# lukeshope/hipims-ocl

Measured on AMD Instinct MI355X. Metric: Mcell-steps/sec fp64 Godunov+HLLC, 4096^2 grid, 1/2/4/8 MI355X; % HBM roofline, higher is better.
Workload: dtype f64

## Files before the change

hipims-ocl_amd/csrc/hp_engine.hip:

```cpp
#include "hp_domain.hpp"
#include "hp_observers.hpp"
#include "hp_actors.hpp"
#include <hip/hip_ext.h>
#include <dlfcn.h>

#include <algorithm>
#include <cmath>
#include <cstdio>
#include <cstdlib>
#include <cstring>
#include <random>
#include <string>
#include <vector>
#include <unistd.h>

namespace {

constexpr size_t CFL_SLOT_BYTES = 1024;

struct Rccl {
	void* handle = nullptr;
	decltype(&ncclGetUniqueId)   GetUniqueId = nullptr;
	decltype(&ncclCommInitRank)  CommInitRank = nullptr;
	decltype(&ncclCommDestroy)   CommDestroy = nullptr;
// ... 2 lines not shown
	decltype(&ncclSend)          Send = nullptr;
	decltype(&ncclRecv)          Recv = nullptr;
	decltype(&ncclAllReduce)     AllReduce = nullptr;
	decltype(&ncclGetErrorString) GetErrorString = nullptr;
	decltype(&ncclCommCount)     CommCount = nullptr;
	std::string path;
} g_rccl;

void peer_release(hp_domain* d);
PeerBox peer_box(hp_domain* d, bool use, long timeout_ms = 0);
PeerPush make_push(const hp_domain* d);

const PlanKnobs& plan_knobs()
{
	static const PlanKnobs knobs = [] {
		auto num = [](const char* name, int unset) { const char* e = std::getenv(name); return e ? std::atoi(e) : unset; };
		auto off = [&](const char* name) { return num(name, 1) == 0; };
		auto on = [&](const char* name) { return num(name, 0) != 0; };
		auto force = [&](const char* name) { return std::getenv(name) ? (num(name, 0) != 0 ? 1 : 0) : -1; };
		PlanKnobs k;
		k.two_step = num("HP_TWO_STEP", -1);
		k.launch_tail = !off("HP_LAUNCH_TAIL"); k.strip_reduce_always = on("HP_STRIP_REDUCE_ALWAYS");
		k.pair_bdy = !off("HP_PAIR_BDY"); k.pair_strict = !off("HP_PAIR_STRICT"); k.pair_exact = force("HP_PAIR_EXACT");
		k.pair_skip = !off("HP_PAIR_SKIP"); k.fill_after_pairs = !off("HP_FILL_AFTER_PAIRS");
		k.strict_speculate = on("HP_STRICT_SPECULATE"); k.pair_tune = !off("HP_PAIR_TUNE"); k.sweep_alternate = force("HP_SWEEP_ALTERNATE");
		k.tail_max_blocks = (unsigned)num("HP_TAIL_MAX_BLOCKS", (int)TAIL_MAX_BLOCKS);
		k.tail_max_blocks_k2k6 = (unsigned)num("HP_TAIL_MAX_BLOCKS_K2K6", (int)TAIL_MAX_BLOCKS);
		k.march2_rseg_forced = std::getenv("HP_MARCH2_RSEG") != nullptr;
		k.fuse_bdy = !off("HP_FUSE_BDY");
		return k;
	}();
	return knobs;
}
PlanDomain plan_domain(const hp_domain* d)
{
	PlanDomain p;
	p.scheme = d->desc.scheme; p.kernel = d->desc.kernel; p.math_mode = d->desc.math_mode; p.precision = d->desc.precision; p.dynamic_dt = d->desc.dynamic_dt;
	p.quirks = d->desc.quirks; p.rows = d->desc.rows; p.cols = d->desc.cols; p.cells = d->cells;
	p.row_offset = d->desc.row_offset; p.global_rows = d->desc.global_rows; p.ghost_rows = d->ghost_rows;
	p.has_bdy = !d->bdy.empty(); p.fusable = d->fusable; p.bdy_on_ring = d->bdy_on_ring;
	for (const Boundary& b : d->bdy)
		if ((b.kind == BDY_UNIFORM && b.definition == HP_UNIFORM_LOSS_RATE) || (b.kind == BDY_GRIDDED && b.definition == HP_GRIDDED_MASS_FLUX)) p.bdy_removes_water = true;
	p.has_comm = d->comm != nullptr; p.comm_world = d->comm_world; p.peer_direct = d->peer_direct; p.peer_mine = d->peer_mine != nullptr;
	p.has_tail_words = d->tail_words != nullptr; p.tail_allowed = d->tail_allowed; p.halo_overlap = d->halo_overlap; p.split_now = d->split_now;
	p.strip_any_bdy = d->strip_any_bdy; p.strip_first = d->strip_first; p.strip_any_full = d->strip_any_full;
	p.spec_now = d->spec_now; p.has_stamps = d->z_state != nullptr; p.march2_pays = d->tiling.march2_pays;
	p.has_links = d->links.groups != 0; p.soil_on = d->soil.on; p.tracer_on = d->tracer.on;
// ... 510 lines not shown
	if ((rc = pair_stamps_alloc(d)) != HP_OK) return rc;
	bool in_place = false;
	if (bdy && !d->facts->m1_valid) {
		if ((rc = pair_cold_start<T>(d)) != HP_OK) return rc;
		in_place = true;
	} else if (bdy) in_place = d->facts->pair_fused_next;
	tail.pair = bdy ? 2 : 1;
	tail.bdy_flag = bdy && followed ? 1 : 0;
	PairAux<T> aux{};
	const bool exact = pair_exact(pd, knobs) && d->z_state != nullptr;
	if (exact) aux.stamps = StampBufs<T>{(char*)d->z_state, d->haz_words};
	aux.prev_gen = d->facts->other_stale ? d->pair_gen : 0u;
	aux.gen = ++d->pair_gen;
	if (aux.gen == 0) aux.gen = ++d->pair_gen;
	aux.list = (const AreaBdyList<T>*)d->fused_list; aux.fuse_next = bdy && followed ? 1 : 0; aux.in_place = in_place ? 1 : 0;
	aux.truncated = (d->desc.quirks & HP_QUIRK_BDY_TRUNCATED) != 0 ? 1 : 0;
	const bool recs = pair_records(pd, knobs, strip, exact, rseg2);
	if (recs) {
		if ((rc = still_rec_alloc(d, tm.nstrips)) != HP_OK) return rc;
		StillRec* const base = (StillRec*)d->still_rec;
		aux.still_out = base + (size_t)(d->still_rec_half ^ 1) * d->still_rec_slots;
		aux.still_in = d->facts->still_rec_valid ? base + (size_t)d->still_rec_half * d->still_rec_slots : nullptr;
		aux.still_rows = d->desc.rows;
	}
	const void* src = d->state[0];
	void* dst = d->state[1];
	const bool sample = d->timing_stride > 0 && d->timing_used < d->timing_events.size() &&
	                    (d->timing_counter++ % (uint64_t)d->timing_stride) == 0;
	if (sample) HIP_TRY(hipEventRecord(d->timing_events[d->timing_used].first, d->stream));
#define HP_LAUNCH_K1B2(CFL_, BDY_, HZ_, TAIL_)                                                                                            \
	hipLaunchKernelGGL((godunov_march2<false, CFL_, BDY_, HZ_, TAIL_, T>), dim3(blocks), dim3(256), 0, d->stream, p, (const Scalars<T>*)d->scalars, \
	                   (const T*)d->bed, (const State4<T>*)src, (State4<T>*)dst, (const T*)d->manning, (T*)d->cfl_slot,                    \
	                   (const T*)d->cfl_slot + SLOT_EDGE, tm, tail, aux)
#define HP_LAUNCH_K1B(CFL_, BDY_, TAIL_) do { if (exact) HP_LAUNCH_K1B2(CFL_, BDY_, true, TAIL_); else HP_LAUNCH_K1B2(CFL_, BDY_, false, TAIL_); } while (0)
	if (d->desc.math_mode == HP_MATH_STRICT)
		hipLaunchKernelGGL((godunov_march2<true, 1, false, true, 1, T>), dim3(blocks), dim3(256), 0, d->stream, p, (const Scalars<T>*)d->scalars,
		                   (const T*)d->bed, (const State4<T>*)src, (State4<T>*)dst, (const T*)d->manning, (T*)d->cfl_slot,
		                   (const T*)d->cfl_slot + SLOT_EDGE, tm, tail, aux);
	else
	if (strip)    { if (d->desc.dynamic_dt) HP_LAUNCH_K1B2(1, false, false, 2); else HP_LAUNCH_K1B2(0, false, false, 2); }
	else if (bdy) HP_LAUNCH_K1B(1, true, 1);
	else          { if (d->desc.dynamic_dt) HP_LAUNCH_K1B(1, false, 1); else HP_LAUNCH_K1B(0, false, 1); }
#undef HP_LAUNCH_K1B
#undef HP_LAUNCH_K1B2
	d->facts.pair_queued(bdy, followed);
	HIP_TRY(hipGetLastError());
// ... 1337 lines not shown
		HIP_TRY(hipEventElapsedTime(&ms, d->timing_events[i].first, d->timing_events[i].second));
		total += std::max(0.0, (double)ms - d->timing_overhead_ms);
		++n;
	}
	*avg_ms = n ? total / n : 0.0;
	*samples = n;
	return HP_OK;
}

int hp_pair_stats(hp_domain_t* d, uint64_t out[12])
{
	int rc = check_domain(d);
	if (rc != HP_OK) return rc;
	if (!out) return fail(HP_ERR_INVALID, "out == NULL");
	out[0] = d->pairs; out[1] = d->pair_cold_starts; out[2] = out[3] = 0;
	HIP_TRY(hipStreamSynchronize(d->stream));
	if (tuner_on(plan_domain(d), plan_knobs()) && (rc = tuner_poll(d)) != HP_OK) return rc;
	out[4] = d->tune_samples; out[5] = d->tune_switches; out[6] = d->tune_prefer_pairs ? 1 : 0;
	out[7] = d->tune_single_ms > 0.f ? (uint64_t)(1000.0 * d->tune_pair_ms / d->tune_single_ms) : 0;
	out[8] = out[9] = out[10] = out[11] = 0;
	if (d->still_rec && d->still_rec_last) {
		const StillRec* half = (const StillRec*)d->still_rec + (size_t)d->still_rec_half * d->still_rec_slots;
		unsigned long long* counts = (unsigned long long*)((StillRec*)d->still_rec + 2 * d->still_rec_slots);
		HIP_TRY(hipMemsetAsync(counts, 0, 16, d->stream));
		hipLaunchKernelGGL(still_rec_count, dim3(256), dim3(256), 0, d->stream, half, d->still_rec_slots, counts);
		HIP_TRY(hipGetLastError());
		unsigned long long host_counts[2] = {0, 0};
		HIP_TRY(hipMemcpyAsync(host_counts, counts, sizeof host_counts, hipMemcpyDeviceToHost, d->stream));
		HIP_TRY(hipStreamSynchronize(d->stream));
		out[9] = host_counts[0]; out[10] = host_counts[1];
	}
	if (d->haz_words) {
		unsigned long long used = 0;
		HIP_TRY(hipMemcpy(&used, d->haz_words + 2, sizeof used, hipMemcpyDeviceToHost));
		out[8] = used;
	}
	if (!d->z_state) return HP_OK;
	unsigned long long* counts = d->haz_words + 4;
	HIP_TRY(hipMemsetAsync(counts, 0, 16, d->stream));
	if (d->desc.precision == 8)
		hipLaunchKernelGGL((stamps_count<double>), dim3(1024), dim3(256), 0, d->stream, StampBufs<double>{(char*)d->z_state, d->haz_words}, d->pair_gen, d->cells, counts);
	else
		hipLaunchKernelGGL((stamps_count<float>), dim3(1024), dim3(256), 0, d->stream, StampBufs<float>{(char*)d->z_state, d->haz_words}, d->pair_gen, d->cells, counts);
	HIP_TRY(hipGetLastError());
	unsigned long long host_counts[2] = {0, 0};
	HIP_TRY(hipMemcpyAsync(host_counts, counts, sizeof host_counts, hipMemcpyDeviceToHost, d->stream));
	HIP_TRY(hipStreamSynchronize(d->stream));
	out[2] = host_counts[0]; out[3] = host_counts[1];
	return HP_OK;
}

int hp_launch_counts(hp_domain_t* d, uint64_t* flux_launches, uint64_t* with_tail)
{
// ... 19 lines not shown
```

hipims-ocl_amd/csrc/hp_kernels.hpp:

```cpp
#pragma once

#include "hp_math.hpp"
#include "hp_tiling.hpp"

namespace hp {

template <bool STRICT, typename T>
__global__ __launch_bounds__(256) void godunov_basic(const Params<T> p, const Scalars<T>* __restrict__ sc,
                                                     const T* __restrict__ bed, const State4<T>* __restrict__ src,
                                                     State4<T>* __restrict__ dst, const T* __restrict__ manning,
                                                     const long y_lo, const long y_hi)
{
	const long x = (long)blockIdx.x * blockDim.x + threadIdx.x;
	const long y = (long)blockIdx.y * blockDim.y + threadIdx.y + y_lo;
	if (x >= p.cols - 1 || y >= y_hi || x <= 0) return;
	const size_t id = (size_t)y * p.cols + x;
	const T dt = sc->dt;

	if (dt <= T(0)) { dst[id] = src[id]; return; }

	const State4<T> c = src[id];
	const T zb = bed[id], n = manning[id];
	if (c.zmax <= T(-9999.0) || c.z == T(-9999.0)) { dst[id] = c; return; }

	const size_t iW = id - 1, iE = id + 1, iS = id - p.cols, iN = id + p.cols;
	const State4<T> cW = src[iW], cE = src[iE], cS = src[iS], cN = src[iN];
// ... 410 lines not shown
}
__device__ __forceinline__ float first_lane(const float v) { return __int_as_float(__builtin_amdgcn_readfirstlane(__float_as_int(v))); }
__device__ __forceinline__ double first_lane(const double v)
{
	return __hiloint2double(__builtin_amdgcn_readfirstlane(__double2hiint(v)), __builtin_amdgcn_readfirstlane(__double2loint(v)));
}
__device__ __forceinline__ unsigned long long value_bits(const double v) { return (unsigned long long)__double_as_longlong(v); }
template <typename V> __device__ __forceinline__ V from_east(const V v) { return lane_move<DPP_WAVE_ROL1>(v); }
template <typename V> __device__ __forceinline__ V from_west(const V v) { return lane_move<DPP_WAVE_ROR1>(v); }

template <typename T> struct RowRegs { State4<T> c; T zb, n; };

template <typename T>
__device__ __forceinline__ Side<T> side_from_east(const Side<T>& s)
{
	Side<T> r;
	r.eta = from_east(s.eta); r.zb = from_east(s.zb);
	r.qx = from_east(s.qx);   r.qy = from_east(s.qy);
	r.u0 = from_east(s.u0);   r.v0 = from_east(s.v0);
	return r;
}


__device__ __forceinline__ bool tile_rows(const TileMap& tm, const int wave, long& strip, long& y0, long& y1)
{
	const unsigned band = blockIdx.x % (unsigned)tm.nbands, i = blockIdx.x / (unsigned)tm.nbands;
	const unsigned nbig_tiles = (unsigned)(tm.groups * tm.nbig);
	const long band_y0 = tm.y_begin + (long)band * tm.band_stride;
	const long band_y1 = (band_y0 + tm.band_rows < tm.y_end) ? (band_y0 + tm.band_rows) : tm.y_end;
	unsigned g;
	long h;
	if (i < nbig_tiles) {
		g = i % (unsigned)tm.groups;
		h = tm.rseg;
		y0 = band_y0 + (long)(i / (unsigned)tm.groups) * tm.rseg;
	} else {
		const unsigned j = i - nbig_tiles;
		g = j % (unsigned)tm.groups;
		h = tm.rseg_tail;
		y0 = band_y0 + (long)tm.nbig * tm.rseg + (long)(j / (unsigned)tm.groups) * tm.rseg_tail;
	}
	y1 = (y0 + h < band_y1) ? (y0 + h) : band_y1;
	strip = (long)g * 4 + wave;
	const bool any = y0 < band_y1 && strip < tm.nstrips;
	if (tm.flip) {
		const long top = band_y0 + (band_y1 - y1);
		y1 = band_y0 + (band_y1 - y0);
		y0 = top;
	}
	return any;
}

template <typename T> struct UniformBdy { const T* series; uint32_t entries; int definition; T interval, length; };
template <typename T> struct GriddedBdy {
	const T* grids; uint64_t entries, grows, gcols; int definition; T resolution, off_x, off_y, interval;
};

template <typename T>
__device__ __forceinline__ bool bdy_in_range(const Params<T>& p, const long x, const long gy, const bool truncated)
{
	if (x >= p.cols - 1 || gy >= p.global_rows - 1 || x <= 0 || gy <= 0) return false;
	if (truncated && (x >= (p.cols / 8) * 8 || gy >= (p.global_rows / 8) * 8)) return false;
	return true;
}

constexpr int AREA_BDY_MAX = 8;
// ... 4 lines not shown
};
template <typename T> struct AreaBdyList { int count; AreaBdy<T> b[AREA_BDY_MAX]; };


constexpr int FUSED_BDY_MAX = 3;
template <typename T> struct FusedBdy {
	T    inc_lo, inc_hi;
	int  y_switch;
	int  mode;
};

template <typename T> constexpr unsigned stamp_rec() { return (unsigned)sizeof(State4<T>) + 16u; }
template <typename T> struct StampBufs { char* rec; unsigned long long* haz; };
template <typename T> __device__ __forceinline__ unsigned stamp_gen(const StampBufs<T>& b, const size_t id)
{
	return *reinterpret_cast<const unsigned*>(b.rec + id * stamp_rec<T>() + sizeof(State4<T>));
}
template <typename T> __device__ __forceinline__ State4<T> stamp_state(const StampBufs<T>& b, const size_t id)
{
	const T* v = reinterpret_cast<const T*>(b.rec + id * stamp_rec<T>());
	State4<T> c; c.z = v[0]; c.zmax = v[1]; c.qx = v[2]; c.qy = v[3];
	return c;
}
struct StillRec { unsigned long long z, b; unsigned tag, pad[3]; };
constexpr unsigned STILL_TAG_RUN = 1, STILL_TAG_SKIP = 2;
template <typename T> struct PairAux {
	StampBufs<T>          stamps;
	unsigned              gen, prev_gen;
	const AreaBdyList<T>* list;
	int                   fuse_next;
	int                   in_place;
	int                   truncated;
	StillRec*             still_out;
	const StillRec*       still_in;
	long                  still_rows;
};

#ifndef HP_K1_STRICT_WAVES
#define HP_K1_STRICT_WAVES 3
#endif
#ifndef HP_K1_FAST_WAVES
#define HP_K1_FAST_WAVES 3
#endif
#ifndef HP_K1_F32_WAVES
#define HP_K1_F32_WAVES 5
#endif
template <bool STRICT, typename T> constexpr int march_waves() { return sizeof(T) == 4 ? HP_K1_F32_WAVES : (STRICT ? HP_K1_STRICT_WAVES : HP_K1_FAST_WAVES); }
// ... 330 lines not shown
template <bool STRICT, int CFL_MODE, bool BDY, bool HZ, int TAIL, typename T>
#ifndef HP_K1B_WAVES_MIN
#define HP_K1B_WAVES_MIN 3
#endif
#ifndef HP_K1B_F32_WAVES_MIN
#define HP_K1B_F32_WAVES_MIN 5
#endif
#ifndef HP_K1B_F32_WAVES_MAX
#define HP_K1B_F32_WAVES_MAX 5
#endif
__global__ __launch_bounds__(256) __attribute__((amdgpu_waves_per_eu(sizeof(T) == 4 ? (STRICT ? 3 : (HZ ? 4 : HP_K1B_F32_WAVES_MIN)) : (STRICT ? HP_K1B_STRICT_WAVES : HP_K1B_WAVES_MIN), sizeof(T) == 4 ? (STRICT ? 3 : HP_K1B_F32_WAVES_MAX) : (STRICT ? HP_K1B_STRICT_WAVES : 3)))) void godunov_march2(
	const Params<T> p, const Scalars<T>* sc, const T* __restrict__ bed, const State4<T>* __restrict__ src,
	State4<T>* __restrict__ dst, const T* __restrict__ manning, T* cfl_slot, const T* __restrict__ edge_max,
	const TileMap tm, const LaunchTail<T> tail, const PairAux<T> aux)
{
	if (TAIL != 0 && blockIdx.x >= tail.flux_blocks) {
		launch_tail(p, tail);
		return;
	}
	__shared__ T inc_tab[BDY ? 4 * 3 * FUSED_BDY_MAX * 2 * 64 : 1];
	const int lane = threadIdx.x & 63, wave = __builtin_amdgcn_readfirstlane((int)(threadIdx.x >> 6));
	long strip, y0, y1;
	T wave_vmax = T(0), wave_vmax1 = T(0);
	if (tile_rows(tm, wave, strip, y0, y1)) {

	const long x = strip * MARCH2_COLS - 1 + lane;
	const long xc = x < 0 ? 0 : (x < p.cols ? x : (p.cols - 1));
	const bool out_x = lane >= 2 && lane <= MARCH2_COLS + 1 && x <= p.cols - 2;
	const bool ring_x = x <= 0 || x >= p.cols - 1;
	const T vs = p.vs;
	const bool with_friction = p.friction != 0;
	const T inv_dx = STRICT ? p.inv_dx_pow2 : p.inv_dx;

	Scalars<T> s1 = *sc;
	const Scalars<T> s0 = s1;
	const T dt_a = s1.dt;
	advance_scalars(p, s1, p.dynamic_dt ? cfl_slot[BDY ? SLOT_M1 : SLOT_SAVED] : T(0));
	const T dt_b = s1.dt;
	const bool skip_a = dt_a <= T(0), skip_b = dt_b <= T(0);
	constexpr bool SCALAR_CONSTS = !STRICT && sizeof(T) == 8;
	constexpr bool HIDE = BDY || HZ;
	const StepConsts<T> ka{uniform_value<HIDE>(-(dt_a * p.inv_dx)), uniform_value<HIDE>(dt_a * gravity<T>()), SCALAR_CONSTS};
	const StepConsts<T> kb{uniform_value<HIDE>(-(dt_b * p.inv_dx)), uniform_value<HIDE>(dt_b * gravity<T>()), SCALAR_CONSTS};

	const long row_base = y0 - 2 < 0 ? 0 : y0 - 2, col_base = strip * MARCH2_COLS - 1 < 0 ? 0 : strip * MARCH2_COLS - 1;
	const size_t cell0 = (size_t)row_base * p.cols + (size_t)col_base;
	const size_t cells_left = (size_t)p.cols * p.rows - cell0;
	const __amdgpu_buffer_rsrc_t srd_src = make_srd(src + cell0, cells_left * sizeof(State4<T>));
	const __amdgpu_buffer_rsrc_t srd_dst = make_srd(dst + cell0, cells_left * sizeof(State4<T>));
	const __amdgpu_buffer_rsrc_t srd_bed = make_srd(bed + cell0, cells_left * sizeof(T));
	const __amdgpu_buffer_rsrc_t srd_man = make_srd(manning + cell0, cells_left * sizeof(T));
	const unsigned lane_col = (unsigned)(xc - col_base);
	const unsigned voff_state = lane_col * (unsigned)sizeof(State4<T>), voff_scalar = lane_col * (unsigned)sizeof(T);
	const unsigned row_state = (unsigned)p.cols * (unsigned)sizeof(State4<T>), row_scalar = (unsigned)p.cols * (unsigned)sizeof(T);
	const long last_row = p.rows - 1;
	const __amdgpu_buffer_rsrc_t srd_peer0 = make_srd((TAIL == 2 && tail.peer_rows[0] ? tail.peer_rows[0] : dst) + cell0, cells_left * sizeof(State4<T>));
	const __amdgpu_buffer_rsrc_t srd_peer1 = make_srd((TAIL == 2 && tail.peer_rows[1] ? tail.peer_rows[1] : dst) + cell0, cells_left * sizeof(State4<T>));
	auto store_peer = [&](const State4<T>& v, const long y, const bool write_lane) {
		const bool e0 = (int)y >= tail.edge_rows[0] && (int)y < tail.edge_rows[1];
		const bool e1 = (int)y >= tail.edge_rows[2] && (int)y < tail.edge_rows[3];
		buf_store_state<HP_AUX_THROUGH>(v, e1 ? srd_peer1 : srd_peer0, (write_lane && (e0 || e1)) ? voff_state : HP_OOB, (unsigned)(y - row_base) * row_state);
	};
	auto load_row = [&](long y, const bool live = true) {
		y = y < 0 ? 0 : (y > last_row ? last_row : y);
		RowRegs<T> r;
		const unsigned k = (unsigned)(y - row_base);
		unsigned vs_ = live ? voff_state : HP_OOB, vc_ = live ? voff_scalar : HP_OOB;
		asm volatile("" : "+v"(vs_), "+v"(vc_));
		r.c = buf_load_state(srd_src, vs_, k * row_state, T());
		r.zb = buf_load_scalar(srd_bed, vc_, k * row_scalar, T());
		r.n = p.manning_uniform ? p.manning_value : buf_load_scalar(srd_man, vc_, k * row_scalar, T());
		return r;
	};
	constexpr bool LAZY_DRY = !STRICT && sizeof(T) == 8;
	auto flux_from_west = [&](const FaceFlux<T>& forW, const bool dryC, bool& dryW) {
		FaceFlux<T> fW;
// ... 68 lines not shown
					if (b.g.definition == 0) {
						inc_lo = rate_lo / T(3600000.0) * thj[j];
						inc_hi = rate_hi / T(3600000.0) * thj[j];
					} else {
						inc_lo = rate_lo / (p.dx * p.dx) * thj[j];
						inc_hi = rate_hi / (p.dx * p.dx) * thj[j];
					}
					ysw[k] = (int)(row_base + n_lo);
					mode = 2u;
				}
				if (mode == 3u) continue;
				tab[((j * FUSED_BDY_MAX + k) * 2 + 0) * 64 + lane] = inc_lo;
				tab[((j * FUSED_BDY_MAX + k) * 2 + 1) * 64 + lane] = inc_hi;
				modes = (modes & ~(3u << (2 * (j * FUSED_BDY_MAX + k)))) | (mode << (2 * (j * FUSED_BDY_MAX + k)));
				act |= 1u << j;
			}
		}
	}
	const bool fuse = BDY && aux.fuse_next != 0;

	T vmax = T(0), vmax1 = T(0);
	unsigned stale_rows = 0;

	constexpr bool RECS = !STRICT && !BDY && !HZ && TAIL == 1 && sizeof(T) == 8;
	unsigned long long still_kz = 0, still_kb = 0;
	unsigned still_marks = 0;
	auto write_recs = [&](const unsigned tag) {
		if (!RECS || aux.still_out == nullptr) return;
		const __amdgpu_buffer_rsrc_t srd = make_srd(aux.still_out + (size_t)strip * aux.still_rows, (size_t)aux.still_rows * sizeof(StillRec));
		const bool m = lane < 32 && ((still_marks >> (unsigned)lane) & 1u) != 0;
		hp_u32x4 a;
		a.x = m ? (unsigned)still_kz : ~0u; a.y = m ? (unsigned)(still_kz >> 32) : ~0u;
		a.z = m ? (unsigned)still_kb : ~0u; a.w = m ? (unsigned)(still_kb >> 32) : ~0u;
		unsigned voff = lane < y1 - y0 ? (unsigned)((y0 + lane) * (long)sizeof(StillRec)) : HP_OOB;
		asm volatile("" : "+v"(voff));
		store_operands_own(a);
		__builtin_amdgcn_raw_buffer_store_b128(a, srd, (int)voff, 0, 0);
		__builtin_amdgcn_raw_buffer_store_b32(m ? tag : 0u, srd, (int)voff + 16, 0, 0);
		store_fence(a, voff, 0u);
	};
	auto tile_known = [&]() -> bool {
		const long xw = strip * MARCH2_COLS - 1;
		if (xw < 1 || xw + 63 > p.cols - 2 || y0 - 2 < 1 || y1 + 1 > last_row - 1 || y1 - y0 > 32) return false;
		const int nr = (int)(y1 - y0) + 4, n = 3 * nr;
		const __amdgpu_buffer_rsrc_t srd = make_srd(aux.still_in + (size_t)(strip - 1) * aux.still_rows, (size_t)3 * aux.still_rows * sizeof(StillRec));
		auto voff = [&](const int i) {
			const int w = i < nr ? 0 : (i < 2 * nr ? 1 : 2);
			return i < n ? (unsigned)(((long)w * aux.still_rows + y0 - 2 + (i - w * nr)) * (long)sizeof(StillRec)) : HP_OOB;
		};
		const hp_u32x4 e0 = __builtin_amdgcn_raw_buffer_load_b128(srd, (int)voff(lane), 0, 0);
		const hp_u32x4 e1 = __builtin_amdgcn_raw_buffer_load_b128(srd, (int)voff(lane + 64), 0, 0);
		const unsigned k0 = __builtin_amdgcn_readfirstlane(e0.x), k1 = __builtin_amdgcn_readfirstlane(e0.y);
		const unsigned k2 = __builtin_amdgcn_readfirstlane(e0.z), k3 = __builtin_amdgcn_readfirstlane(e0.w);
		if (k0 == ~0u && k1 == ~0u) return false;
		auto same = [&](const hp_u32x4& e) { return e.x == k0 && e.y == k1 && e.z == k2 && e.w == k3; };
		if (!wave_all((lane >= n || same(e0)) && (lane + 64 >= n || same(e1)))) return false;
		still_kz = ((unsigned long long)k1 << 32) | k0;
		still_kb = ((unsigned long long)k3 << 32) | k2;
		return true;
	};

// ... 275 lines not shown
			buf_store_state(c, srd_dst, out_x ? voff_state : HP_OOB, row_k * row_state);
			if (TAIL == 2) store_peer(c, yy, out_x);
			if (CFL_MODE == 1 && out_x && (int)yy >= tm.price_lo && (int)yy < tm.price_hi && spd > vmax) vmax = spd;
		};
		State4<T> a = q[2].c, b = q[3].c;
		for (;;) {
			if (y >= y1) return y;
			#pragma unroll
			for (int j = 0; j < 4; ++j) q[j] = load_rz(y + 2 + j);
			if (!in_run(q[0])) return y;
			put(a, y);
			if (y + 1 >= y1 || !in_run(q[1])) return y + 1;
			put(b, y + 1);
			if (y + 2 >= y1 || !in_run(q[2])) return y + 2;
			put(q[0].c, y + 2);
			if (y + 3 >= y1 || !in_run(q[3])) return y + 3;
			put(q[1].c, y + 3);
			a = q[2].c; b = q[3].c;
			y += 4;
		}
	};

	const long yb = (RUNS && !skip_a && !skip_b) ? still_run() : y0;
	write_recs(STILL_TAG_RUN);
	if (!RUNS || yb < y1) {
		prime(yb);
		long r = yb + 1;
		for (; r + 1 <= y1; r += 2) {
			{ const T nn = rc.n; const RowU1<T> u = stage_a(r, rP, rQ); stage_b(r - 1, u, nn, true); }
			{ const T nn = rc.n; const RowU1<T> u = stage_a(r + 1, rQ, rP); stage_b(r, u, nn, true); }
		}
		if (r <= y1) { const T nn = rc.n; const RowU1<T> u = stage_a(r, rP, rQ); stage_b(r - 1, u, nn, true); }
	}

	if (wave_any(stale_rows != 0)) {
		for (long y = y0; y < y1; ++y) {
			if ((stale_rows >> (unsigned)(y - y0)) & 1u) {
				const size_t id = (size_t)y * p.cols + xc;
				const T zb = bed[id];
				State4<T> c = src[id];
				if (live0) c = apply(J0(), c, zb, y);
				State4<T> next = c;
				if (live2) next = apply(J2(), c, zb, y);
				dst[id] = fuse ? next : c;
				if (TAIL == 2) store_peer(fuse ? next : c, y, true);
				if (CFL_MODE == 1 && (int)y >= tm.price_lo && (int)y < tm.price_hi) {
					const T s = cfl_speed<STRICT>(c.z, c.zmax, c.qx, c.qy, zb, p.qs);
					if (s > vmax) vmax = s;
					if (live2) {
						const T s2 = cfl_speed<STRICT>(next.z, next.zmax, next.qx, next.qy, zb, p.qs);
						if (s2 > vmax1) vmax1 = s2;
					}
				}
			}
		}
	}
	if (!live2) vmax1 = vmax;
	};

	auto raise_word = [&]() { if (hz_on && wave_any(stamped) && lane == 0) aux.stamps.haz[aux.gen & 1u] = (unsigned long long)aux.gen; };
	if (RECS && aux.still_in != nullptr && !skip_a && !skip_b && tile_known()) {
		still_marks = ~0u;
		write_recs(STILL_TAG_SKIP);
		if (CFL_MODE == 1 && out_x && (int)y1 > tm.price_lo && (int)y0 < tm.price_hi)
			vmax = cfl_speed<STRICT>(T(__longlong_as_double((long long)still_kz)), T(0), T(0), T(0), T(__longlong_as_double((long long)still_kb)), p.qs);
		vmax1 = vmax;
	} else {
	if (BDY && act != 0) { if (hz_any) march(std::true_type(), std::true_type()); else march(std::true_type(), std::false_type()); }
	else                 { if (hz_any) march(std::false_type(), std::true_type()); else march(std::false_type(), std::false_type()); }
	raise_word();
	}

	if (CFL_MODE != 0) {
		if (blockIdx.x == 0 && wave == 0) { const T e = *edge_max; if (e > vmax) vmax = e; if (e > vmax1) vmax1 = e; }
		vmax = wave_max(vmax);
		if (BDY) vmax1 = wave_max(vmax1);
		if (TAIL != 0) { wave_vmax = vmax; wave_vmax1 = vmax1; }
		else if (lane == 0 && vmax > T(0)) atomic_max_nonneg(cfl_slot, vmax);
	}
	}
	if (TAIL != 0) tail_block_done<BDY>(tail, wave_vmax, wave, lane, y0, y1, wave_vmax1);
}

template <typename T>
__global__ __launch_bounds__(256) void stamps_to_buffer(State4<T>* __restrict__ other, const StampBufs<T> b, const unsigned gen, const size_t cells)
{
	if (b.haz[gen & 1u] != (unsigned long long)gen) return;
	for (size_t id = (size_t)blockIdx.x * blockDim.x + threadIdx.x; id < cells; id += (size_t)gridDim.x * blockDim.x)
		if (stamp_gen(b, id) == gen) other[id] = stamp_state(b, id);
}

template <typename T>
__global__ __launch_bounds__(256) void stamps_count(const StampBufs<T> b, const unsigned gen, const size_t cells, unsigned long long* counts)
{
	unsigned long long last = 0, any = 0;
	for (size_t id = (size_t)blockIdx.x * blockDim.x + threadIdx.x; id < cells; id += (size_t)gridDim.x * blockDim.x) {
		const unsigned g = stamp_gen(b, id);
		last += (g != 0 && g == gen); any += (g != 0);
	}
	for (int off = 32; off > 0; off >>= 1) { last += __shfl_down(last, off); any += __shfl_down(any, off); }
	if ((threadIdx.x & 63) == 0 && (last | any)) { atomicAdd(counts, last); atomicAdd(counts + 1, any); }
}
__global__ __launch_bounds__(256) void still_rec_count(const StillRec* __restrict__ rec, const size_t n, unsigned long long* counts)
{
	unsigned long long skipped = 0, still = 0;
	for (size_t i = (size_t)blockIdx.x * blockDim.x + threadIdx.x; i < n; i += (size_t)gridDim.x * blockDim.x) {
		const unsigned tag = rec[i].tag;
		skipped += (tag == STILL_TAG_SKIP); still += (tag == STILL_TAG_SKIP || tag == STILL_TAG_RUN);
	}
	for (int off = 32; off > 0; off >>= 1) { skipped += __shfl_down(skipped, off); still += __shfl_down(still, off); }
	if ((threadIdx.x & 63) == 0 && (skipped | still)) { atomicAdd(counts, skipped); atomicAdd(counts + 1, still); }
}

template <typename T>
__global__ void pair_cold_start_words(T* slot)
{
	slot[SLOT_M1] = atomic_exchange_zero(slot);
	slot[SLOT_BDY] = T(1);
}

template <typename T>
__global__ __launch_bounds__(256) void rings_compare(const State4<T>* __restrict__ a, const State4<T>* __restrict__ b, const long cols, const long rows,
                                                     unsigned long long* differ)
{
	const long n = 2 * cols + 2 * (rows - 2);
	bool bad = false;
	for (long i = (long)blockIdx.x * blockDim.x + threadIdx.x; i < n; i += (long)gridDim.x * blockDim.x) {
		long x, y;
		if (i < cols) { x = i; y = 0; }
		else if (i < 2 * cols) { x = i - cols; y = rows - 1; }
		else { const long j = i - 2 * cols; x = (j & 1) ? cols - 1 : 0; y = 1 + (j >> 1); }
		const size_t id = (size_t)y * cols + x;
		const unsigned* wa = reinterpret_cast<const unsigned*>(a + id);
		const unsigned* wb = reinterpret_cast<const unsigned*>(b + id);
// ... 606 lines not shown
```

hipims-ocl_amd/csrc/hp_plan.hpp:

```cpp
#pragma once
#include "../../include/hipims_mi.h"
#include "hp_facts.hpp"

#include <algorithm>
#include <cstddef>
#include <cstdint>

namespace hp {
namespace {

constexpr unsigned TAIL_MAX_BLOCKS = 65536;
constexpr uint32_t SPEC_MIN = 8;

struct PlanKnobs {
	int      two_step = -1;
	bool     launch_tail = true;
	bool     strip_reduce_always = false;
	bool     pair_bdy = true;
	bool     pair_strict = true;
	int      pair_exact = -1;
	bool     pair_skip = true;
	bool     fill_after_pairs = true;
	bool     strict_speculate = false;
	bool     pair_tune = true;
	int      sweep_alternate = -1;
	unsigned tail_max_blocks = TAIL_MAX_BLOCKS;
	unsigned tail_max_blocks_k2k6 = TAIL_MAX_BLOCKS;
	bool     march2_rseg_forced = false;
	bool     fuse_bdy = true;
};

struct PlanDomain {
	int      scheme = HP_SCHEME_GODUNOV, kernel = HP_KERNEL_AUTO, math_mode = HP_MATH_FAST, precision = 8, dynamic_dt = 1;
	unsigned quirks = HP_QUIRKS_REFERENCE;
	long     rows = 0, cols = 0;
	size_t   cells = 0;
	long     row_offset = 0, global_rows = 0, ghost_rows = 1;
	bool     has_bdy = false;
	bool     fusable = false, bdy_on_ring = false;
	bool     bdy_removes_water = false;
	bool     has_comm = false;
	int      comm_world = 1;
	bool     peer_direct = false, peer_mine = false;
	bool     has_tail_words = true, tail_allowed = false, halo_overlap = false, split_now = true;
// ... 42 lines not shown
}
inline bool pair_eligible(const PlanDomain& d, const BufferFacts& facts, const PlanKnobs& k)
{
	return pairs_possible(d, k) && facts.pair_ready(d.dynamic_dt != 0);
}
inline bool strip_pairs_possible_here(const PlanDomain& d, const BufferFacts& facts, const PlanKnobs& k)
{
	return pairs_possible_common(d, k) && d.has_comm && d.comm_world > 1 && d.peer_direct && d.ghost_rows == 2 && !facts->rings_differ;
}
inline bool pair_exact(const PlanDomain& d, const PlanKnobs& k)
{
	if (d.math_mode == HP_MATH_STRICT) return true;
	if (k.pair_exact >= 0) return k.pair_exact != 0;
	return d.bdy_removes_water;
}
inline int pair_tile_rows(const PlanDomain& d, const PlanKnobs& k, const int march2_rseg)
{
	return (d.math_mode == HP_MATH_STRICT && !k.march2_rseg_forced) ? std::min(march2_rseg, 12) : march2_rseg;
}
inline bool pair_records(const PlanDomain& d, const PlanKnobs& k, const bool strip, const bool exact, const int tile_rows)
{
	return d.precision == 8 && k.pair_skip && !strip && !d.has_bdy && !exact && d.math_mode != HP_MATH_STRICT && tile_rows <= 32;
}

inline bool fill_wanted(const PlanDomain& d, const BufferFacts& facts, const PlanKnobs& k)
{
	return k.fill_after_pairs && facts->other_stale && d.scheme == HP_SCHEME_GODUNOV && d.kernel != HP_KERNEL_BASIC && !(pair_exact(d, k) && d.has_stamps);
}

inline bool spec_wanted(const PlanDomain& d, const PlanKnobs& k, const uint32_t n)
{
	const bool fusable_ok = d.spec_fused_kept || !d.fusable;
	return k.strict_speculate && n >= SPEC_MIN && d.math_mode == HP_MATH_STRICT && d.precision == 8 && !d.has_comm && fusable_ok && !d.has_links && !d.soil_on && !d.tracer_on &&
	       d.kernel != HP_KERNEL_BASIC && (d.scheme == HP_SCHEME_GODUNOV || d.scheme == HP_SCHEME_MUSCL_HANCOCK);
}
inline bool tuner_on(const PlanDomain& d, const PlanKnobs& k)
{
	return k.pair_tune && d.math_mode == HP_MATH_STRICT && k.two_step != 1;
}

inline bool strips_reduce_everyone(const PlanDomain& d, const BufferFacts& facts, const bool first_of_batch)
{
	const bool dst_is_primary = facts->use_alt == 1;
	return d.dynamic_dt && (d.scheme == HP_SCHEME_MUSCL_HANCOCK || !reads_primary(d) || dst_is_primary || basic_godunov(d) || d.strip_any_bdy ||
	                        (first_of_batch && d.strip_any_full));
}
// ... 44 lines not shown
```

hipims-ocl_amd/csrc/hp_tiling.hpp:

```cpp
#pragma once
#include <algorithm>
#include <cstdlib>
#include <initializer_list>
#include <vector>

namespace hp {

constexpr int MARCH_COLS = 62;
constexpr int MARCH2_COLS = 60;
constexpr int MUSCL_COLS = 60;

struct TileMap {
	int  nstrips, groups;
	long y_begin, y_end;
	int  nbands;
	long band_stride;
	int  band_rows;
	int  rseg, nbig;
	int  rseg_tail, ntail;
	int  price_lo, price_hi;
	int  flip;
};

struct TilingKnobs {
	bool   rseg_refine = true;
	bool   search = true, search_pair = true;
	bool   search_f32 = false;
	double tiling_fill = 3.5, march2_fill = 4.0;
	int    march_rseg = 0, muscl_rseg = 0, inertial_rseg = 0, march2_rseg = 0;
	int    tail_rseg = 0, tail_pct = -1;
	bool   print_tiling = false;
};
struct LaunchKnobs {
	long   halo_rows = 0;
	int    nbands = 0;
};

struct Tiling {
// ... 127 lines not shown
{
	Tiling t = pick_tiling(cols, rows, precision, cus, knobs);
	force_heights(t, knobs);
	return t;
}

inline bool tiles_addressable(const Tiling& t, const long cols, const int precision)
{
	const int rseg_max = std::max(std::max(t.march_rseg, t.march2_rseg), std::max(t.muscl_rseg, t.inertial_rseg));
	return (double)(rseg_max + 4) * (double)cols * 4.0 * (double)precision < 2147483647.0;
}

enum { PART_ALL = 0, PART_HALO = 1, PART_INTERIOR = 2 };

struct RowRange { long lo, hi; };

inline bool make_tile_map(const LaunchKnobs& knobs, long lo, long hi, int g, int part, int nstrips, int rseg, int rseg_tail, int tail_pct,
                          TileMap& tm, unsigned& blocks, int rseg_tall = 16, long need = 0, long price_lo = 0, long price_hi = 0x7fffffffL,
                          int nbands = 8)
{
	if (need < g) need = g;
	const long halo = knobs.halo_rows >= need ? knobs.halo_rows : (rseg > need ? rseg : need);
	tm.price_lo = (int)price_lo; tm.price_hi = (int)(price_hi < 0x7fffffffL ? price_hi : 0x7fffffffL);
	tm.flip = 0;
	const bool can_split = hi - lo > 2 * halo;
	tm.nstrips = nstrips;
	tm.groups = (nstrips + 3) / 4;
	if (part == PART_HALO && can_split) {
		tm.y_begin = lo; tm.y_end = hi;
		tm.nbands = 2; tm.band_stride = (hi - halo) - lo; tm.band_rows = (int)halo;
		tm.rseg = rseg < tm.band_rows ? rseg : tm.band_rows;
		tm.nbig = (tm.band_rows + tm.rseg - 1) / tm.rseg;
		tm.rseg_tail = rseg_tail; tm.ntail = 0;
		blocks = 2u * (unsigned)(tm.groups * tm.nbig);
		return true;
	}
	if (part == PART_INTERIOR) {
		if (!can_split) return false;
		lo += halo; hi -= halo;
	}
	tm.y_begin = lo; tm.y_end = hi;
	const long rows = hi - lo;
	tm.nbands = part != PART_ALL ? 8 : (knobs.nbands >= 1 && knobs.nbands <= 64 ? knobs.nbands : (nbands >= 1 && nbands <= 64 ? nbands : 8));
	tm.band_rows = (int)((rows + tm.nbands - 1) / tm.nbands);
	tm.band_stride = tm.band_rows;
	if (rseg == 16 && g == 1 && tm.band_rows >= 256) rseg = rseg_tall;
	tm.rseg = rseg < tm.band_rows ? rseg : tm.band_rows;
// ... 16 lines not shown
```

hipims-ocl_amd/hipims_mi/__init__.py:

```python
from __future__ import annotations

import ctypes as C
import os
import weakref

import numpy as np

HERE = os.path.dirname(os.path.abspath(__file__))
PKG_ROOT = os.path.dirname(HERE)
LIB_PATH = os.path.join(PKG_ROOT, "lib", "libhipims_mi.so")

SCHEME_GODUNOV, SCHEME_MUSCL_HANCOCK, SCHEME_INERTIAL = 0, 1, 2
ARRAY_STATE, ARRAY_BED, ARRAY_MANNING = 0, 1, 2
QUIRK_CFL_READS_PRIMARY, QUIRK_BDY_TRUNCATED, QUIRK_MUSCL_NEIGHBOUR_Y_IS_BED, QUIRKS_REFERENCE = 1, 2, 4, 7
MATH_FAST, MATH_STRICT = 0, 1
KERNEL_AUTO, KERNEL_BASIC = 0, 1
UNIFORM_RAIN_INTENSITY, UNIFORM_LOSS_RATE = 0, 1
GRIDDED_RAIN_INTENSITY, GRIDDED_RAIN_ACCUMUL, GRIDDED_MASS_FLUX = 0, 1, 2
DEPTH_IGNORE, DEPTH_IS_FSL, DEPTH_IS_DEPTH, DEPTH_IS_CRITICAL = 0, 1, 2, 3
DISCHARGE_IGNORE, DISCHARGE_IS_DISCHARGE, DISCHARGE_IS_VELOCITY, DISCHARGE_IS_VOLUME = 0, 1, 2, 3
PTR_STATE_NEXT_SRC, PTR_STATE_OTHER, PTR_BED, PTR_MANNING, PTR_CFL_MAX, PTR_SCALARS = range(6)
(OUT_DEPTH, OUT_MAXDEPTH, OUT_FSL, OUT_MAXFSL, OUT_DISCHARGE_X, OUT_DISCHARGE_Y, OUT_VELOCITY_X, OUT_VELOCITY_Y, OUT_FROUDE,
 OUT_COUNT) = range(10)
OUT_CODES = {"depth": OUT_DEPTH, "maxdepth": OUT_MAXDEPTH, "fsl": OUT_FSL, "maxfsl": OUT_MAXFSL, "dischargex": OUT_DISCHARGE_X,
# ... 1067 lines not shown
    def kernel_timing(self, stride):
        _check(self.lib, self.lib.hp_kernel_timing(self.h, stride), "hp_kernel_timing")

    def kernel_timing_read(self):
        avg, n = C.c_double(0), C.c_uint32(0)
        _check(self.lib, self.lib.hp_kernel_timing_read(self.h, C.byref(avg), C.byref(n)), "hp_kernel_timing_read")
        return avg.value, n.value

    def launch_counts(self):
        if not hasattr(self.lib, "hp_launch_counts"):
            return None
        a, b = C.c_uint64(0), C.c_uint64(0)
        _check(self.lib, self.lib.hp_launch_counts(self.h, C.byref(a), C.byref(b)), "hp_launch_counts")
        return a.value, b.value

    def pair_stats(self):
        if not hasattr(self.lib, "hp_pair_stats"):
            return None
        out = (C.c_uint64 * 12)()
        self.lib.hp_pair_stats.argtypes = [C.c_void_p, C.POINTER(C.c_uint64)]
        _check(self.lib, self.lib.hp_pair_stats(self.h, out), "hp_pair_stats")
        return dict(pairs=out[0], cold_starts=out[1], stamped_last=out[2], stamped_ever=out[3], tune_samples=out[4],
                    tune_switches=out[5], prefers_pairs=bool(out[6]), pair_over_single=out[7] / 1000.0, stale_used=out[8],
                    skipped_rows=out[9], still_rows=out[10])

    def kernel_timing_overhead(self):
        if not hasattr(self.lib, "hp_kernel_timing_overhead"):
            return 0.0
        ms = C.c_double(0)
        _check(self.lib, self.lib.hp_kernel_timing_overhead(self.h, C.byref(ms)), "hp_kernel_timing_overhead")
        return ms.value

    def depth_velocity(self, state=None, bed=None):
        state = self.download() if state is None else state
        bed = self._bed_host if bed is None else bed
        depth = np.maximum(0.0, state[..., 0].astype(np.float64) - bed.astype(np.float64))
        with np.errstate(divide="ignore", invalid="ignore"):
            u = np.where(depth > 1e-8, state[..., 2] / depth, 0.0)
            v = np.where(depth > 1e-8, state[..., 3] / depth, 0.0)
        return depth, u, v
```

Measured before the change: 122,100.

## Redeal idle waves onto still-marching tiles within a block for skip pairs

When still-water skip records are active, strips are assigned to a block's four waves with a stride instead of contiguously. Waves whose tile was skipped take a share of the rows of the one or two waves that still have to march, splitting those rows into parts of at least three rows. The aim is to cut the load imbalance where a block waits on a single wave marching a full tile. It adds shared-memory flags, extra __syncthreads, recomputed buffer descriptors and a dealt counter in the still records, and it disables still-run marks for split parts, which may cost some skipping.

New measurement: 118,700. 0.972x the previous value.

```diff
diff --git a/hipims-ocl_amd/csrc/hp_engine.hip b/hipims-ocl_amd/csrc/hp_engine.hip
--- a/hipims-ocl_amd/csrc/hp_engine.hip
+++ b/hipims-ocl_amd/csrc/hp_engine.hip
@@ -48,7 +48,7 @@
 		k.two_step = num("HP_TWO_STEP", -1);
 		k.launch_tail = !off("HP_LAUNCH_TAIL"); k.strip_reduce_always = on("HP_STRIP_REDUCE_ALWAYS");
 		k.pair_bdy = !off("HP_PAIR_BDY"); k.pair_strict = !off("HP_PAIR_STRICT"); k.pair_exact = force("HP_PAIR_EXACT");
-		k.pair_skip = !off("HP_PAIR_SKIP"); k.fill_after_pairs = !off("HP_FILL_AFTER_PAIRS");
+		k.pair_skip = !off("HP_PAIR_SKIP"); k.pair_redeal = !off("HP_PAIR_REDEAL"); k.fill_after_pairs = !off("HP_FILL_AFTER_PAIRS");
 		k.strict_speculate = on("HP_STRICT_SPECULATE"); k.pair_tune = !off("HP_PAIR_TUNE"); k.sweep_alternate = force("HP_SWEEP_ALTERNATE");
 		k.tail_max_blocks = (unsigned)num("HP_TAIL_MAX_BLOCKS", (int)TAIL_MAX_BLOCKS);
 		k.tail_max_blocks_k2k6 = (unsigned)num("HP_TAIL_MAX_BLOCKS_K2K6", (int)TAIL_MAX_BLOCKS);
@@ -605,6 +605,7 @@
 		aux.still_out = base + (size_t)(d->still_rec_half ^ 1) * d->still_rec_slots;
 		aux.still_in = d->facts->still_rec_valid ? base + (size_t)d->still_rec_half * d->still_rec_slots : nullptr;
 		aux.still_rows = d->desc.rows;
+		if (pair_redeal(knobs, recs)) tm.stride = tm.groups;
 	}
 	const void* src = d->state[0];
 	void* dst = d->state[1];
@@ -1988,13 +1989,13 @@
 	if (d->still_rec && d->still_rec_last) {
 		const StillRec* half = (const StillRec*)d->still_rec + (size_t)d->still_rec_half * d->still_rec_slots;
 		unsigned long long* counts = (unsigned long long*)((StillRec*)d->still_rec + 2 * d->still_rec_slots);
-		HIP_TRY(hipMemsetAsync(counts, 0, 16, d->stream));
+		HIP_TRY(hipMemsetAsync(counts, 0, 24, d->stream));
 		hipLaunchKernelGGL(still_rec_count, dim3(256), dim3(256), 0, d->stream, half, d->still_rec_slots, counts);
 		HIP_TRY(hipGetLastError());
-		unsigned long long host_counts[2] = {0, 0};
+		unsigned long long host_counts[3] = {0, 0, 0};
 		HIP_TRY(hipMemcpyAsync(host_counts, counts, sizeof host_counts, hipMemcpyDeviceToHost, d->stream));
 		HIP_TRY(hipStreamSynchronize(d->stream));
-		out[9] = host_counts[0]; out[10] = host_counts[1];
+		out[9] = host_counts[0]; out[10] = host_counts[1]; out[11] = host_counts[2];
 	}
 	if (d->haz_words) {
 		unsigned long long used = 0;
diff --git a/hipims-ocl_amd/csrc/hp_kernels.hpp b/hipims-ocl_amd/csrc/hp_kernels.hpp
--- a/hipims-ocl_amd/csrc/hp_kernels.hpp
+++ b/hipims-ocl_amd/csrc/hp_kernels.hpp
@@ -2,6 +2,7 @@
 
 #include "hp_math.hpp"
 #include "hp_tiling.hpp"
+#include "hp_redeal.hpp"
 
 namespace hp {
 
@@ -458,6 +459,7 @@
 }
 
 
+template <bool STRIDED = false>
 __device__ __forceinline__ bool tile_rows(const TileMap& tm, const int wave, long& strip, long& y0, long& y1)
 {
 	const unsigned band = blockIdx.x % (unsigned)tm.nbands, i = blockIdx.x / (unsigned)tm.nbands;
@@ -477,7 +479,7 @@
 		y0 = band_y0 + (long)tm.nbig * tm.rseg + (long)(j / (unsigned)tm.groups) * tm.rseg_tail;
 	}
 	y1 = (y0 + h < band_y1) ? (y0 + h) : band_y1;
-	strip = (long)g * 4 + wave;
+	strip = (STRIDED && tm.stride != 0) ? (long)g + (long)wave * tm.stride : (long)g * 4 + wave;
 	const bool any = y0 < band_y1 && strip < tm.nstrips;
 	if (tm.flip) {
 		const long top = band_y0 + (band_y1 - y1);
@@ -528,7 +530,7 @@
 	State4<T> c; c.z = v[0]; c.zmax = v[1]; c.qx = v[2]; c.qy = v[3];
 	return c;
 }
-struct StillRec { unsigned long long z, b; unsigned tag, pad[3]; };
+struct StillRec { unsigned long long z, b; unsigned tag, dealt, pad[2]; };
 constexpr unsigned STILL_TAG_RUN = 1, STILL_TAG_SKIP = 2;
 template <typename T> struct PairAux {
 	StampBufs<T>          stamps;
@@ -905,12 +907,21 @@
 	const int lane = threadIdx.x & 63, wave = __builtin_amdgcn_readfirstlane((int)(threadIdx.x >> 6));
 	long strip, y0, y1;
 	T wave_vmax = T(0), wave_vmax1 = T(0);
-	if (tile_rows(tm, wave, strip, y0, y1)) {
-
-	const long x = strip * MARCH2_COLS - 1 + lane;
-	const long xc = x < 0 ? 0 : (x < p.cols ? x : (p.cols - 1));
-	const bool out_x = lane >= 2 && lane <= MARCH2_COLS + 1 && x <= p.cols - 2;
-	const bool ring_x = x <= 0 || x >= p.cols - 1;
+	constexpr bool RECS = !STRICT && !BDY && !HZ && TAIL == 1 && sizeof(T) == 8;
+	__shared__ unsigned redeal_words[RECS ? 4 + 16 : 1];
+	const bool have_tile = tile_rows<RECS>(tm, wave, strip, y0, y1);
+	const bool redeal_on = RECS && tm.stride != 0;
+	if (have_tile || redeal_on) {
+
+	long x, xc;
+	bool out_x, ring_x;
+	auto place_columns = [&]() {
+		x = strip * MARCH2_COLS - 1 + lane;
+		xc = x < 0 ? 0 : (x < p.cols ? x : (p.cols - 1));
+		out_x = lane >= 2 && lane <= MARCH2_COLS + 1 && x <= p.cols - 2;
+		ring_x = x <= 0 || x >= p.cols - 1;
+	};
+	place_columns();
 	const T vs = p.vs;
 	const bool with_friction = p.friction != 0;
 	const T inv_dx = STRICT ? p.inv_dx_pow2 : p.inv_dx;
@@ -926,15 +937,22 @@
 	const StepConsts<T> ka{uniform_value<HIDE>(-(dt_a * p.inv_dx)), uniform_value<HIDE>(dt_a * gravity<T>()), SCALAR_CONSTS};
 	const StepConsts<T> kb{uniform_value<HIDE>(-(dt_b * p.inv_dx)), uniform_value<HIDE>(dt_b * gravity<T>()), SCALAR_CONSTS};
 
-	const long row_base = y0 - 2 < 0 ? 0 : y0 - 2, col_base = strip * MARCH2_COLS - 1 < 0 ? 0 : strip * MARCH2_COLS - 1;
-	const size_t cell0 = (size_t)row_base * p.cols + (size_t)col_base;
-	const size_t cells_left = (size_t)p.cols * p.rows - cell0;
-	const __amdgpu_buffer_rsrc_t srd_src = make_srd(src + cell0, cells_left * sizeof(State4<T>));
-	const __amdgpu_buffer_rsrc_t srd_dst = make_srd(dst + cell0, cells_left * sizeof(State4<T>));
-	const __amdgpu_buffer_rsrc_t srd_bed = make_srd(bed + cell0, cells_left * sizeof(T));
-	const __amdgpu_buffer_rsrc_t srd_man = make_srd(manning + cell0, cells_left * sizeof(T));
-	const unsigned lane_col = (unsigned)(xc - col_base);
-	const unsigned voff_state = lane_col * (unsigned)sizeof(State4<T>), voff_scalar = lane_col * (unsigned)sizeof(T);
+	long row_base, col_base;
+	size_t cell0, cells_left;
+	__amdgpu_buffer_rsrc_t srd_src, srd_dst, srd_bed, srd_man;
+	unsigned lane_col, voff_state, voff_scalar;
+	auto place_window = [&]() {
+		row_base = y0 - 2 < 0 ? 0 : y0 - 2; col_base = strip * MARCH2_COLS - 1 < 0 ? 0 : strip * MARCH2_COLS - 1;
+		cell0 = (size_t)row_base * p.cols + (size_t)col_base;
+		cells_left = (size_t)p.cols * p.rows - cell0;
+		srd_src = make_srd(src + cell0, cells_left * sizeof(State4<T>));
+		srd_dst = make_srd(dst + cell0, cells_left * sizeof(State4<T>));
+		srd_bed = make_srd(bed + cell0, cells_left * sizeof(T));
+		srd_man = make_srd(manning + cell0, cells_left * sizeof(T));
+		lane_col = (unsigned)(xc - col_base);
+		voff_state = lane_col * (unsigned)sizeof(State4<T>); voff_scalar = lane_col * (unsigned)sizeof(T);
+	};
+	place_window();
 	const unsigned row_state = (unsigned)p.cols * (unsigned)sizeof(State4<T>), row_scalar = (unsigned)p.cols * (unsigned)sizeof(T);
 	const long last_row = p.rows - 1;
 	const __amdgpu_buffer_rsrc_t srd_peer0 = make_srd((TAIL == 2 && tail.peer_rows[0] ? tail.peer_rows[0] : dst) + cell0, cells_left * sizeof(State4<T>));
@@ -1049,9 +1067,10 @@
 	T vmax = T(0), vmax1 = T(0);
 	unsigned stale_rows = 0;
 
-	constexpr bool RECS = !STRICT && !BDY && !HZ && TAIL == 1 && sizeof(T) == 8;
 	unsigned long long still_kz = 0, still_kb = 0;
 	unsigned still_marks = 0;
+	unsigned redealt = 0;
+	int part_slot = 0, part_index = 0;
 	auto write_recs = [&](const unsigned tag) {
 		if (!RECS || aux.still_out == nullptr) return;
 		const __amdgpu_buffer_rsrc_t srd = make_srd(aux.still_out + (size_t)strip * aux.still_rows, (size_t)aux.still_rows * sizeof(StillRec));
@@ -1064,6 +1083,7 @@
 		store_operands_own(a);
 		__builtin_amdgcn_raw_buffer_store_b128(a, srd, (int)voff, 0, 0);
 		__builtin_amdgcn_raw_buffer_store_b32(m ? tag : 0u, srd, (int)voff + 16, 0, 0);
+		__builtin_amdgcn_raw_buffer_store_b32(redealt, srd, (int)voff + 20, 0, 0);
 		store_fence(a, voff, 0u);
 	};
 	auto tile_known = [&]() -> bool {
@@ -1385,6 +1405,11 @@
 	};
 
 	const long yb = (RUNS && !skip_a && !skip_b) ? still_run() : y0;
+	if (redeal_on) {
+		if (lane == 0) redeal_words[4 + 4 * part_slot + part_index] = yb >= y1 ? 1u : 0u;
+		__syncthreads();
+		for (int j = 0; j < part_index; ++j) if (redeal_words[4 + 4 * part_slot + j] == 0u) still_marks = 0;
+	}
 	write_recs(STILL_TAG_RUN);
 	if (!RUNS || yb < y1) {
 		prime(yb);
@@ -1422,17 +1447,42 @@
 	};
 
 	auto raise_word = [&]() { if (hz_on && wave_any(stamped) && lane == 0) aux.stamps.haz[aux.gen & 1u] = (unsigned long long)aux.gen; };
-	if (RECS && aux.still_in != nullptr && !skip_a && !skip_b && tile_known()) {
+	bool marches = have_tile;
+	if (RECS && have_tile && aux.still_in != nullptr && !skip_a && !skip_b && tile_known()) {
 		still_marks = ~0u;
 		write_recs(STILL_TAG_SKIP);
 		if (CFL_MODE == 1 && out_x && (int)y1 > tm.price_lo && (int)y0 < tm.price_hi)
 			vmax = cfl_speed<STRICT>(T(__longlong_as_double((long long)still_kz)), T(0), T(0), T(0), T(__longlong_as_double((long long)still_kb)), p.qs);
 		vmax1 = vmax;
-	} else {
+		marches = false;
+	}
+	if (redeal_on) {
+		part_slot = wave;
+		if (lane == 0) redeal_words[wave] = (marches ? 1u : 0u) | (have_tile ? 2u : 0u);
+		__syncthreads();
+		if (aux.still_in != nullptr && !skip_a && !skip_b) {
+			unsigned needy = 0, present = 0;
+			for (int w = 0; w < 4; ++w) {
+				const unsigned f = (unsigned)__builtin_amdgcn_readfirstlane((int)redeal_words[w]);
+				needy |= (f & 1u) << (unsigned)w; present |= ((f >> 1) & 1u) << (unsigned)w;
+			}
+			const RedealPart part = redeal_part(needy, present, wave, y0, y1);
+			marches = part.slot >= 0;
+			if (marches && part.parts > 1) {
+				strip += (long)(part.slot - wave) * tm.stride;
+				y0 = part.y0; y1 = part.y1;
+				part_slot = part.slot; part_index = part.part;
+				redealt = 1u; still_marks = 0;
+				place_columns();
+				place_window();
+			}
+		}
+	}
+	if (marches) {
 	if (BDY && act != 0) { if (hz_any) march(std::true_type(), std::true_type()); else march(std::true_type(), std::false_type()); }
 	else                 { if (hz_any) march(std::false_type(), std::true_type()); else march(std::false_type(), std::false_type()); }
 	raise_word();
-	}
+	} else if (redeal_on) __syncthreads();
 
 	if (CFL_MODE != 0) {
 		if (blockIdx.x == 0 && wave == 0) { const T e = *edge_max; if (e > vmax) vmax = e; if (e > vmax1) vmax1 = e; }
@@ -1466,13 +1516,14 @@
 }
 __global__ __launch_bounds__(256) void still_rec_count(const StillRec* __restrict__ rec, const size_t n, unsigned long long* counts)
 {
-	unsigned long long skipped = 0, still = 0;
+	unsigned long long skipped = 0, still = 0, dealt = 0;
 	for (size_t i = (size_t)blockIdx.x * blockDim.x + threadIdx.x; i < n; i += (size_t)gridDim.x * blockDim.x) {
 		const unsigned tag = rec[i].tag;
 		skipped += (tag == STILL_TAG_SKIP); still += (tag == STILL_TAG_SKIP || tag == STILL_TAG_RUN);
-	}
-	for (int off = 32; off > 0; off >>= 1) { skipped += __shfl_down(skipped, off); still += __shfl_down(still, off); }
-	if ((threadIdx.x & 63) == 0 && (skipped | still)) { atomicAdd(counts, skipped); atomicAdd(counts + 1, still); }
+		dealt += (rec[i].dealt == 1u);
+	}
+	for (int off = 32; off > 0; off >>= 1) { skipped += __shfl_down(skipped, off); still += __shfl_down(still, off); dealt += __shfl_down(dealt, off); }
+	if ((threadIdx.x & 63) == 0 && (skipped | still | dealt)) { atomicAdd(counts, skipped); atomicAdd(counts + 1, still); atomicAdd(counts + 2, dealt); }
 }
 
 template <typename T>
diff --git a/hipims-ocl_amd/csrc/hp_plan.hpp b/hipims-ocl_amd/csrc/hp_plan.hpp
--- a/hipims-ocl_amd/csrc/hp_plan.hpp
+++ b/hipims-ocl_amd/csrc/hp_plan.hpp
@@ -20,6 +20,7 @@
 	bool     pair_strict = true;
 	int      pair_exact = -1;
 	bool     pair_skip = true;
+	bool     pair_redeal = true;
 	bool     fill_after_pairs = true;
 	bool     strict_speculate = false;
 	bool     pair_tune = true;
@@ -108,6 +109,7 @@
 {
 	return d.precision == 8 && k.pair_skip && !strip && !d.has_bdy && !exact && d.math_mode != HP_MATH_STRICT && tile_rows <= 32;
 }
+inline bool pair_redeal(const PlanKnobs& k, const bool records) { return k.pair_redeal && records; }
 
 inline bool fill_wanted(const PlanDomain& d, const BufferFacts& facts, const PlanKnobs& k)
 {
diff --git a/hipims-ocl_amd/csrc/hp_redeal.hpp b/hipims-ocl_amd/csrc/hp_redeal.hpp
--- /dev/null
+++ b/hipims-ocl_amd/csrc/hp_redeal.hpp
@@ -0,0 +1,47 @@
+#pragma once
+
+#ifndef HP_HOST_DEVICE
+#if defined(__HIPCC__) || defined(__CUDACC__)
+#define HP_HOST_DEVICE __host__ __device__
+#else
+#define HP_HOST_DEVICE
+#endif
+#endif
+
+namespace hp {
+
+constexpr int REDEAL_MIN_ROWS = 3;
+
+struct RedealPart { int slot; long y0, y1; int part, parts; };
+
+HP_HOST_DEVICE inline RedealPart redeal_part(const unsigned needy_mask, const unsigned present_mask, const int wave, const long y0, const long y1)
+{
+	const unsigned needy = needy_mask & present_mask & 15u;
+	const unsigned me = 1u << (unsigned)wave;
+	const RedealPart own = {(needy & me) ? wave : -1, y0, y1, 0, 1};
+	int count = 0;
+	for (int w = 0; w < 4; ++w) count += (int)((needy >> (unsigned)w) & 1u);
+	if (count != 1 && count != 2) return own;
+	const long h = y1 - y0;
+	const int share = count == 1 ? 4 : 2;
+	const int parts = (int)(h / REDEAL_MIN_ROWS) < share ? (int)(h / REDEAL_MIN_ROWS) : share;
+	if (parts < 2) return own;
+	int slot = -1, part = 0;
+	if (needy & me) slot = wave;
+	else {
+		int idle_rank = 0;
+		for (int w = 0; w < wave; ++w) idle_rank += (int)(((needy >> (unsigned)w) & 1u) ^ 1u);
+		int first = 0;
+		while (!((needy >> (unsigned)first) & 1u)) ++first;
+		int second = first + 1;
+		while (second < 4 && !((needy >> (unsigned)second) & 1u)) ++second;
+		if (count == 1) { slot = first; part = 1 + idle_rank; }
+		else            { slot = idle_rank == 0 ? first : second; part = 1; }
+		if (part >= parts) return own;
+	}
+	const long base = h / parts, rem = h % parts;
+	const long lo = y0 + (long)part * base + ((long)part < rem ? (long)part : rem);
+	return RedealPart{slot, lo, lo + base + ((long)part < rem ? 1 : 0), part, parts};
+}
+
+}
diff --git a/hipims-ocl_amd/csrc/hp_tiling.hpp b/hipims-ocl_amd/csrc/hp_tiling.hpp
--- a/hipims-ocl_amd/csrc/hp_tiling.hpp
+++ b/hipims-ocl_amd/csrc/hp_tiling.hpp
@@ -14,6 +14,7 @@
 	int  nstrips, groups;
 	long y_begin, y_end;
 	int  nbands;
+	int  stride;
 	long band_stride;
 	int  band_rows;
 	int  rseg, nbig;
@@ -187,7 +188,7 @@
 	if (need < g) need = g;
 	const long halo = knobs.halo_rows >= need ? knobs.halo_rows : (rseg > need ? rseg : need);
 	tm.price_lo = (int)price_lo; tm.price_hi = (int)(price_hi < 0x7fffffffL ? price_hi : 0x7fffffffL);
-	tm.flip = 0;
+	tm.flip = 0; tm.stride = 0;
 	const bool can_split = hi - lo > 2 * halo;
 	tm.nstrips = nstrips;
 	tm.groups = (nstrips + 3) / 4;
diff --git a/hipims-ocl_amd/hipims_mi/__init__.py b/hipims-ocl_amd/hipims_mi/__init__.py
--- a/hipims-ocl_amd/hipims_mi/__init__.py
+++ b/hipims-ocl_amd/hipims_mi/__init__.py
@@ -1113,7 +1113,7 @@
         _check(self.lib, self.lib.hp_pair_stats(self.h, out), "hp_pair_stats")
         return dict(pairs=out[0], cold_starts=out[1], stamped_last=out[2], stamped_ever=out[3], tune_samples=out[4],
                     tune_switches=out[5], prefers_pairs=bool(out[6]), pair_over_single=out[7] / 1000.0, stale_used=out[8],
-                    skipped_rows=out[9], still_rows=out[10])
+                    skipped_rows=out[9], still_rows=out[10], redealt_rows=out[11])
 
     def kernel_timing_overhead(self):
         if not hasattr(self.lib, "hp_kernel_timing_overhead"):
```
